# showlab/VideoSwap

Hardware: NVIDIA H100
Metric: denoise-steps/sec, 16f 512^2 SD1.5 UNet3D (CFG UNet fwd + CFG combine + DDIM step) (higher is better)
Workload: dtype f16

## Files before the change

### videoswap_b200/csrc/common.cuh

```cuda
#pragma once
#include <cuda.h>
#include <cuda_fp16.h>
#include <cuda_runtime.h>
#include <stdint.h>
#include <stdio.h>

namespace vs {

void set_error(const char* fmt, ...);
const char* last_error();

#define VS_CHECK_CUDA(expr)                                                                         \
  do {                                                                                              \
    cudaError_t _e = (expr);                                                                        \
    if (_e != cudaSuccess) {                                                                        \
      vs::set_error("%s:%d CUDA error %s: %s", __FILE__, __LINE__, #expr, cudaGetErrorString(_e)); \
      return 1;                                                                                     \
    }                                                                                               \
  } while (0)

#define VS_REQUIRE(cond, ...)                \
  do {                                       \
    if (!(cond)) {                           \
      vs::set_error(__VA_ARGS__);            \
      return 2;                              \
    }                                        \
  } while (0)

int make_tmap_f16(CUtensorMap* out, const void* base, int rank, const uint64_t* dims, const uint64_t* strides_bytes,
                  const uint32_t* box, int swizzle );

int num_sms();
int get_option(const char* name);

#ifdef __CUDACC__
template <typename... KArgs, typename... Args>
int launch_pdl(void (*kernel)(KArgs...), dim3 grid, dim3 block, size_t smem, cudaStream_t st, int cluster_x, Args&&... args) {
  cudaLaunchConfig_t cfg = {};
  cfg.gridDim = grid;
  cfg.blockDim = block;
  cfg.dynamicSmemBytes = smem;
  cfg.stream = st;
  cudaLaunchAttribute attr[2];
  int n = 0;
  if (get_option("pdl") != 0) {
    attr[n].id = cudaLaunchAttributeProgrammaticStreamSerialization;
    attr[n].val.programmaticStreamSerializationAllowed = 1;
    ++n;
  }
  if (cluster_x > 1) {
    attr[n].id = cudaLaunchAttributeClusterDimension;
    attr[n].val.clusterDim.x = cluster_x;
    attr[n].val.clusterDim.y = 1;
    attr[n].val.clusterDim.z = 1;
    ++n;
  }
  cfg.attrs = attr;
  cfg.numAttrs = n;
  VS_CHECK_CUDA(cudaLaunchKernelEx(&cfg, kernel, static_cast<KArgs>(args)...));
  return 0;
}
#endif

enum ProfCat { PC_GEMM = 0, PC_CONV = 1, PC_ATTN = 2, PC_TATTN = 3, PC_GROUPNORM = 4, PC_LAYERNORM = 5, PC_OTHER = 6, PC_COUNT = 7 };
struct ProfScope {
  ProfScope(cudaStream_t st, int cat, double work, int nlaunch = 1, long long m = 0, int n = 0, int k = 0);
  ~ProfScope();
  cudaStream_t st_; int idx_;
};
void prof_enable(bool on);
void prof_reset();
int prof_collect(int cat, double* ms, double* work, long long* count);
int prof_dump(const char* path);
long long launch_count();
void count_launch(int n);

#ifdef __CUDACC__
__device__ __forceinline__ uint32_t smem_u32(const void* p) { return (uint32_t)__cvta_generic_to_shared(p); }

__device__ __forceinline__ void mbar_init(uint32_t bar, uint32_t count) {
  asm volatile("mbarrier.init.shared::cta.b64 [%0], %1;" ::"r"(bar), "r"(count) : "memory");
}
__device__ __forceinline__ void fence_barrier_init() {
  asm volatile("fence.mbarrier_init.release.cluster;" ::: "memory");
}
__device__ __forceinline__ void fence_proxy_async() { asm volatile("fence.proxy.async.shared::cta;" ::: "memory"); }
__device__ __forceinline__ void mbar_expect_tx(uint32_t bar, uint32_t bytes) {
  asm volatile("mbarrier.arrive.expect_tx.shared::cta.b64 _, [%0], %1;" ::"r"(bar), "r"(bytes) : "memory");
}
__device__ __forceinline__ void mbar_arrive(uint32_t bar) {
  asm volatile("mbarrier.arrive.shared::cta.b64 _, [%0];" ::"r"(bar) : "memory");
}
__device__ __forceinline__ bool mbar_try_wait(uint32_t bar, uint32_t parity) {
  uint32_t ok;
  asm volatile(
      "{\n\t.reg .pred p;\n\t"
      "mbarrier.try_wait.parity.shared::cta.b64 p, [%1], %2;\n\t"
      "selp.u32 %0, 1, 0, p;\n\t}"
      : "=r"(ok)
      : "r"(bar), "r"(parity)
      : "memory");
  return ok != 0;
}
__device__ __forceinline__ void mbar_wait(uint32_t bar, uint32_t parity) {
  if (mbar_try_wait(bar, parity)) return;
  uint32_t spins = 0;
  while (!mbar_try_wait(bar, parity)) {
    if (++spins > (1u << 25)) __trap();
  }
}

__device__ __forceinline__ void prefetch_tmap(const CUtensorMap* m) {
  asm volatile("prefetch.tensormap [%0];" ::"l"(reinterpret_cast<uint64_t>(m)) : "memory");
}
__device__ __forceinline__ void tma_load_2d(uint32_t dst, const CUtensorMap* m, uint32_t bar, int c0, int c1) {
  asm volatile(
      "cp.async.bulk.tensor.2d.shared::cluster.global.mbarrier::complete_tx::bytes [%0], [%1, {%3, %4}], [%2];"
      ::"r"(dst), "l"(reinterpret_cast<uint64_t>(m)), "r"(bar), "r"(c0), "r"(c1)
      : "memory");
}
__device__ __forceinline__ void tma_load_4d(uint32_t dst, const CUtensorMap* m, uint32_t bar, int c0, int c1, int c2,
                                            int c3) {
  asm volatile(
      "cp.async.bulk.tensor.4d.shared::cluster.global.mbarrier::complete_tx::bytes [%0], [%1, {%3, %4, %5, %6}], [%2];"
      ::"r"(dst), "l"(reinterpret_cast<uint64_t>(m)), "r"(bar), "r"(c0), "r"(c1), "r"(c2), "r"(c3)
      : "memory");
}

__device__ __forceinline__ bool elect_one() {
  uint32_t pred;
  asm volatile(
      "{\n\t.reg .pred P;\n\t"
      "elect.sync _|P, 0xffffffff;\n\t"
      "selp.u32 %0, 1, 0, P;\n\t}"
      : "=r"(pred));
  return pred != 0;
}

__device__ __forceinline__ uint32_t cluster_ctarank() {
  uint32_t r;
  asm volatile("mov.u32 %0, %%cluster_ctarank;" : "=r"(r));
  return r;
}
__device__ __forceinline__ void cluster_sync_all() {
  asm volatile("barrier.cluster.arrive.release.aligned;" ::: "memory");
  asm volatile("barrier.cluster.wait.acquire.aligned;" ::: "memory");
}
__device__ __forceinline__ uint32_t mapa_shared(uint32_t addr, uint32_t rank) {
  uint32_t r;
  asm volatile("mapa.shared::cluster.u32 %0, %1, %2;" : "=r"(r) : "r"(addr), "r"(rank));
  return r;
}
__device__ __forceinline__ void named_bar_sync(int id, int nthreads) {
  asm volatile("bar.sync %0, %1;" ::"r"(id), "r"(nthreads) : "memory");
}
__device__ __forceinline__ void named_bar_arrive(int id, int nthreads) {
  asm volatile("bar.arrive %0, %1;" ::"r"(id), "r"(nthreads) : "memory");
}

__device__ __forceinline__ void pdl_trigger() { asm volatile("griddepcontrol.launch_dependents;" ::: "memory"); }
__device__ __forceinline__ void pdl_wait() { asm volatile("griddepcontrol.wait;" ::: "memory"); }

template <int N>
__device__ __forceinline__ void setmaxnreg_dec() { asm volatile("setmaxnreg.dec.sync.aligned.u32 %0;" ::"n"(N)); }
template <int N>
__device__ __forceinline__ void setmaxnreg_inc() { asm volatile("setmaxnreg.inc.sync.aligned.u32 %0;" ::"n"(N)); }

__device__ __forceinline__ void wgmma_fence() { asm volatile("wgmma.fence.sync.aligned;" ::: "memory"); }
__device__ __forceinline__ void wgmma_commit() { asm volatile("wgmma.commit_group.sync.aligned;" ::: "memory"); }
template <int N>
__device__ __forceinline__ void wgmma_wait() { asm volatile("wgmma.wait_group.sync.aligned %0;" ::"n"(N) : "memory"); }

__device__ __forceinline__ uint64_t gmma_desc_sw128(uint32_t smem_addr) {
  uint64_t d = 0;
  d |= (uint64_t)((smem_addr & 0x3FFFF) >> 4);
  d |= (uint64_t)1 << 16;
  d |= (uint64_t)(1024 >> 4) << 32;
  d |= (uint64_t)1 << 62;
  return d;
}
__device__ __forceinline__ uint64_t gmma_desc_sw128_mn(uint32_t smem_addr, uint32_t lbo_bytes) {
  uint64_t d = 0;
  d |= (uint64_t)((smem_addr & 0x3FFFF) >> 4);
  d |= (uint64_t)((lbo_bytes >> 4) & 0x3FFF) << 16;
  d |= (uint64_t)(1024 >> 4) << 32;
  d |= (uint64_t)1 << 62;
  return d;
}

#define VS_R8(i) "+f"(d[i]), "+f"(d[i + 1]), "+f"(d[i + 2]), "+f"(d[i + 3]), "+f"(d[i + 4]), "+f"(d[i + 5]), "+f"(d[i + 6]), "+f"(d[i + 7])
template <int N>
__device__ __forceinline__ void wgmma_ss(float* d, uint64_t da, uint64_t db, uint32_t scale_d);
#define VS_REGS_0_31 "%0,%1,%2,%3,%4,%5,%6,%7,%8,%9,%10,%11,%12,%13,%14,%15,%16,%17,%18,%19,%20,%21,%22,%23,%24,%25,%26,%27,%28,%29,%30,%31"
#define VS_REGS_32_63 "%32,%33,%34,%35,%36,%37,%38,%39,%40,%41,%42,%43,%44,%45,%46,%47,%48,%49,%50,%51,%52,%53,%54,%55,%56,%57,%58,%59,%60,%61,%62,%63"
#define VS_REGS_64_79 "%64,%65,%66,%67,%68,%69,%70,%71,%72,%73,%74,%75,%76,%77,%78,%79"
#define VS_REGS_80_127 "%80,%81,%82,%83,%84,%85,%86,%87,%88,%89,%90,%91,%92,%93,%94,%95,%96,%97,%98,%99,%100,%101,%102,%103,%104,%105,%106,%107,%108,%109,%110,%111,%112,%113,%114,%115,%116,%117,%118,%119,%120,%121,%122,%123,%124,%125,%126,%127"
#define VS_WGMMA_SS(N, REGS, IA, IB, IS, ...)                                                                     \
  template <>                                                                                                     \
  __device__ __forceinline__ void wgmma_ss<N>(float* d, uint64_t da, uint64_t db, uint32_t scale_d) {           \
    asm volatile("{\n\t.reg .pred p;\n\tsetp.ne.b32 p, %" #IS ", 0;\n\t"                                         \
                 "wgmma.mma_async.sync.aligned.m64n" #N "k16.f32.f16.f16 {" REGS "}, %" #IA ", %" #IB ", p, 1, 1, 0, 0;\n\t}" \
                 : __VA_ARGS__                                                                                    \
                 : "l"(da), "l"(db), "r"(scale_d));                                                               \
  }
VS_WGMMA_SS(64, VS_REGS_0_31, 32, 33, 34, VS_R8(0), VS_R8(8), VS_R8(16), VS_R8(24))
VS_WGMMA_SS(128, VS_REGS_0_31 "," VS_REGS_32_63, 64, 65, 66, VS_R8(0), VS_R8(8), VS_R8(16), VS_R8(24), VS_R8(32), VS_R8(40),
            VS_R8(48), VS_R8(56))
VS_WGMMA_SS(160, VS_REGS_0_31 "," VS_REGS_32_63 "," VS_REGS_64_79, 80, 81, 82, VS_R8(0), VS_R8(8), VS_R8(16), VS_R8(24),
            VS_R8(32), VS_R8(40), VS_R8(48), VS_R8(56), VS_R8(64), VS_R8(72))
VS_WGMMA_SS(256, VS_REGS_0_31 "," VS_REGS_32_63 "," VS_REGS_64_79 "," VS_REGS_80_127, 128, 129, 130, VS_R8(0), VS_R8(8),
            VS_R8(16), VS_R8(24), VS_R8(32), VS_R8(40), VS_R8(48), VS_R8(56), VS_R8(64), VS_R8(72), VS_R8(80), VS_R8(88),
            VS_R8(96), VS_R8(104), VS_R8(112), VS_R8(120))
#undef VS_WGMMA_SS
#undef VS_REGS_0_31
#undef VS_REGS_32_63
#undef VS_REGS_64_79
#undef VS_REGS_80_127
template <int TB = 0>
__device__ __forceinline__ void wgmma_m64n16(float* d, uint64_t da, uint64_t db, uint32_t scale_d) {
  asm volatile(
      "{\n\t.reg .pred p;\n\tsetp.ne.b32 p, %10, 0;\n\t"
      "wgmma.mma_async.sync.aligned.m64n16k16.f32.f16.f16 {%0,%1,%2,%3,%4,%5,%6,%7}, %8, %9, p, 1, 1, 0, %11;\n\t}"
      : VS_R8(0)
      : "l"(da), "l"(db), "r"(scale_d), "n"(TB));
}
template <int TB = 0>
__device__ __forceinline__ void wgmma_m64n64_rs(float* d, const uint32_t* a, uint64_t db, uint32_t scale_d) {
  asm volatile(
      "{\n\t.reg .pred p;\n\tsetp.ne.b32 p, %37, 0;\n\t"
      "wgmma.mma_async.sync.aligned.m64n64k16.f32.f16.f16 "
      "{%0,%1,%2,%3,%4,%5,%6,%7,%8,%9,%10,%11,%12,%13,%14,%15,%16,%17,%18,%19,%20,%21,%22,%23,%24,%25,%26,%27,%28,%29,%30,%31}, "
      "{%32,%33,%34,%35}, %36, p, 1, 1, %38;\n\t}"
      : VS_R8(0), VS_R8(8), VS_R8(16), VS_R8(24)
      : "r"(a[0]), "r"(a[1]), "r"(a[2]), "r"(a[3]), "l"(db), "r"(scale_d), "n"(TB));
}
template <int TB = 0>
__device__ __forceinline__ void wgmma_m64n16_rs(float* d, const uint32_t* a, uint64_t db, uint32_t scale_d) {
  asm volatile(
      "{\n\t.reg .pred p;\n\tsetp.ne.b32 p, %13, 0;\n\t"
      "wgmma.mma_async.sync.aligned.m64n16k16.f32.f16.f16 {%0,%1,%2,%3,%4,%5,%6,%7}, {%8,%9,%10,%11}, %12, p, 1, 1, %14;\n\t}"
      : VS_R8(0)
      : "r"(a[0]), "r"(a[1]), "r"(a[2]), "r"(a[3]), "l"(db), "r"(scale_d), "n"(TB));
}
#undef VS_R8

__device__ __forceinline__ float silu_f(float x) { return __fdividef(x, 1.f + __expf(-x)); }
__device__ __forceinline__ float gelu_erf_f(float x) { return 0.5f * x * (1.f + erff(x * 0.70710678118654752f)); }
__device__ __forceinline__ float gelu_erf_fast(float x) {
  const float z = fabsf(x) * 0.70710678118654752f;
  float t;
  asm("rcp.approx.ftz.f32 %0, %1;" : "=f"(t) : "f"(fmaf(0.3275911f, z, 1.f)));
  float poly = fmaf(1.061405429f, t, -1.453152027f);
  poly = fmaf(poly, t, 1.421413741f);
  poly = fmaf(poly, t, -0.284496736f);
  poly = fmaf(poly, t, 0.254829592f);
  poly *= t;
  float e;
  asm("ex2.approx.ftz.f32 %0, %1;" : "=f"(e) : "f"(-1.4426950408889634f * z * z));
  const float erf_abs = fmaf(-poly, e, 1.f);
  const float erf_s = copysignf(erf_abs, x);
  return 0.5f * x * (1.f + erf_s);
}
__device__ __forceinline__ float gelu_sig(float x) {
  const float xc = fminf(fmaxf(x, -5.f), 5.f);
  const float u = xc * xc;
  float q = fmaf(u, 2.47135360e-05f, 7.37690930e-04f);
  q = fmaf(q, u, -1.05988323e-01f);
  q = fmaf(q, u, -2.30164247e+00f);
  float e;
  asm("ex2.approx.ftz.f32 %0, %1;" : "=f"(e) : "f"(xc * q));
  return __fdividef(x, 1.f + e);
}
#endif

}
```

### videoswap_b200/csrc/gemm.cu

```cuda
#include "common.cuh"
#include "kernels.h"

namespace vs {

namespace {

constexpr int BM = 128;
constexpr int WG_M = 64;
constexpr int BK = 64;
constexpr int A_STAGE_BYTES = BM * BK * 2;
constexpr uint64_t A_HALF_DESC = (WG_M * BK * 2) >> 4;
constexpr int GEMM_THREADS = 384;
constexpr int SMEM_LIMIT = 227 * 1024;
constexpr int EPI_COLS = 32;
constexpr int EPI_WARP_BYTES = 16 * 64;
constexpr int EPI_BYTES = 8 * EPI_WARP_BYTES;
constexpr int PRODUCER_REGS = 40, CONSUMER_REGS = 232;
enum { EPI_F_GEGLU = 1, EPI_F_RES = 2, EPI_F_RV = 4, EPI_F_LN = 8, EPI_F_LNOUT = 16 };

struct GemmParams {
  CUtensorMap tmA, tmA2, tmB;
  int M, N;
  int num_kb;
  int kb_per_tap;
  int kb_src1;
  int taps;
  int a_rank;
  int nimg, H, W, TH, TW, TN, tiles_x, tiles_y;
  int tap_x0, tap_y0, tap_w;
  int osy, osx, ooy, oox, OH, OW;
  int tw_log, thw_log;
  int m_tiles, n_tiles;
  const float* bias;
  const float* rowvec;
  int ldrv;
  int pix_per_batch;
  int rv_mod;
  const float2* ln_stats;
  const float* ln_u;
  const float2* ln_parts;
  int ln_nparts;
  float ln_inv_c;
  float2* ln_sums_out;
  const __half* residual;
  int ldr;
  __half* out;
  int ldc;
  int staged;
  int stages;
};

template <int BN>
struct Cfg {
  static constexpr bool COOP = BN > 160;
  static constexpr int HALVES = COOP ? 1 : 2;
  static constexpr int B_STAGE_BYTES = BN * BK * 2;
  static constexpr int STAGE_BYTES = A_STAGE_BYTES + B_STAGE_BYTES;
  static constexpr int STAGES_RAW = (SMEM_LIMIT - 2048 - EPI_BYTES) / STAGE_BYTES;
  static constexpr int STAGES = STAGES_RAW > 12 ? 12 : STAGES_RAW;
  static constexpr int SMEM_BYTES = STAGES * STAGE_BYTES + EPI_BYTES + 1024  + 256 ;
  static_assert(B_STAGE_BYTES % 1024 == 0, "B stage must keep 1024-byte alignment for SWIZZLE_128B");
  static_assert(STAGES >= 3, "pipeline too shallow");
  static_assert(BN % 32 == 0 && BN <= 256, "wgmma N");
};

__device__ __forceinline__ uint32_t sw64_off(int row, int chunk) {
  return (uint32_t)(row * 64 + ((chunk ^ ((row >> 1) & 3)) << 4));
}

template <int BN, int EPI>
__global__ void __launch_bounds__(GEMM_THREADS, 1) gemm_tc_kernel(const __grid_constant__ GemmParams p) {
  using C = Cfg<BN>;
  constexpr bool GEGLU = (EPI & EPI_F_GEGLU) != 0, HAS_RES = (EPI & EPI_F_RES) != 0, HAS_RV = (EPI & EPI_F_RV) != 0;
  constexpr bool LN = (EPI & EPI_F_LN) != 0;
  constexpr bool LNOUT = (EPI & EPI_F_LNOUT) != 0;
  extern __shared__ uint8_t smem_raw[];
  const uint32_t smem_base = (smem_u32(smem_raw) + 1023u) & ~1023u;
  const uint32_t epi_base = smem_base + C::STAGES * C::STAGE_BYTES;
  const uint32_t bar_base = epi_base + EPI_BYTES;
  auto full_bar = [&](int s) { return bar_base + 8u * s; };
  auto empty_bar = [&](int s) { return bar_base + 8u * (C::STAGES + s); };

  const int warp = threadIdx.x >> 5;
  const int lane = threadIdx.x & 31;
  const int wg = threadIdx.x >> 7;
  const int nst = (p.stages > 0 && p.stages < C::STAGES) ? p.stages : C::STAGES;
  const int total_tiles = p.m_tiles * p.n_tiles;

  if (threadIdx.x == 0) {
    prefetch_tmap(&p.tmA);
    prefetch_tmap(&p.tmB);
    if (p.kb_src1 < p.kb_per_tap) prefetch_tmap(&p.tmA2);
    for (int s = 0; s < C::STAGES; ++s) {
      mbar_init(full_bar(s), 1);
      mbar_init(empty_bar(s), C::COOP ? 8 : 4);
    }
    fence_barrier_init();
  }
  __syncthreads();
  pdl_trigger();
  pdl_wait();

  if (wg == 0) {
    setmaxnreg_dec<PRODUCER_REGS>();
    if (warp != 0) return;
    const int num_kb = p.num_kb, kb_per_tap = p.kb_per_tap, kb_src1 = p.kb_src1;
    const bool conv = p.a_rank == 4;
    const int tap_x0 = p.tap_x0, tap_x1 = p.tap_x0 + p.tap_w;
    uint32_t pr_s = 0, pr_ph = 0;
    for (int t = blockIdx.x; t < total_tiles; t += gridDim.x) {
      const int m_tile = t / p.n_tiles, n_tile = t % p.n_tiles;
      int x0 = 0, y0 = 0, i0 = 0;
      if (conv) {
        x0 = (m_tile % p.tiles_x) * p.TW;
        y0 = ((m_tile / p.tiles_x) % p.tiles_y) * p.TH;
        i0 = (m_tile / (p.tiles_x * p.tiles_y)) * p.TN;
      }
      const int n0 = n_tile * BN;
      const int m0 = m_tile * BM;
      int kcoord = 0;
      int dy = p.tap_y0, dx = tap_x0;
      int r = 0;
      for (int kb = 0; kb < num_kb; ++kb) {
        mbar_wait(empty_bar(pr_s), pr_ph ^ 1);
        if (elect_one()) {
          const uint32_t fb = full_bar(pr_s);
          const uint32_t a_dst = smem_base + pr_s * C::STAGE_BYTES;
          const bool first = r < kb_src1;
          const CUtensorMap* tm = first ? &p.tmA : &p.tmA2;
          const int c = (first ? r : r - kb_src1) * BK;
          mbar_expect_tx(fb, C::STAGE_BYTES);
          if (conv) tma_load_4d(a_dst, tm, fb, c, x0 + dx, y0 + dy, i0);
          else tma_load_2d(a_dst, tm, fb, c, m0);
          tma_load_2d(a_dst + A_STAGE_BYTES, &p.tmB, fb, kcoord, n0);
        }
        __syncwarp();
        kcoord += BK;
        if (++r == kb_per_tap) {
          r = 0;
          if (++dx == tap_x1) { dx = tap_x0; ++dy; }
        }
        if (++pr_s == (uint32_t)nst) { pr_s = 0; pr_ph ^= 1; }
      }
    }
    return;
  }

  setmaxnreg_inc<CONSUMER_REGS>();
  const int g = wg - 1;
  const int wq = warp & 3;
  const int q = lane & 3;
  const int rbase = 16 * wq + (lane >> 2);
  const uint32_t stage_buf = epi_base + (uint32_t)(warp - 4) * EPI_WARP_BYTES;
  const bool has_bias = p.bias != nullptr;
  const bool staged = p.staged != 0;
  const int num_kb = p.num_kb;
  auto tile_pixel = [&](int m_tile, int row) -> int {
    if (p.a_rank == 4) {
      const int x0 = (m_tile % p.tiles_x) * p.TW;
      const int y0 = ((m_tile / p.tiles_x) % p.tiles_y) * p.TH;
      const int i0 = (m_tile / (p.tiles_x * p.tiles_y)) * p.TN;
      const int ti = row >> p.thw_log, rem = row & ((1 << p.thw_log) - 1);
      const int y = y0 + (rem >> p.tw_log), x = x0 + (rem & (p.TW - 1)), img = i0 + ti;
      return ((img < p.nimg) && (y < p.H) && (x < p.W)) ? (img * p.OH + y * p.osy + p.ooy) * p.OW + x * p.osx + p.oox : -1;
    }
    const int px = m_tile * BM + row;
    return px < p.M ? px : -1;
  };

  const int bar_mine = 1 + g, bar_other = 2 - g;
  float acc[C::HALVES][BN / 2];
  uint32_t s = 0, ph = 0;
  for (int t = blockIdx.x, j = 0; t < total_tiles; t += gridDim.x, ++j) {
    const int m_tile = t / p.n_tiles, n_tile = t % p.n_tiles;
    if (!C::COOP && (j & 1) != g) {
      const uint32_t sn = s + (uint32_t)num_kb;
      ph ^= (sn / (uint32_t)nst) & 1u;
      s = sn % (uint32_t)nst;
      continue;
    }
    if (!C::COOP && j > 0) named_bar_sync(bar_mine, 256);
    uint32_t prev = 0;
    for (int kb = 0; kb < num_kb; ++kb) {
      mbar_wait(full_bar(s), ph);
      wgmma_fence();
      const uint32_t a_addr = smem_base + s * C::STAGE_BYTES;
      const uint64_t da = gmma_desc_sw128(a_addr) + (C::COOP ? (uint64_t)g * A_HALF_DESC : 0);
      const uint64_t db = gmma_desc_sw128(a_addr + A_STAGE_BYTES);
#pragma unroll
      for (int k = 0; k < BK / 16; ++k) {
#pragma unroll
        for (int hh = 0; hh < C::HALVES; ++hh)
          wgmma_ss<BN>(acc[hh], da + hh * A_HALF_DESC + 2 * k, db + 2 * k, (kb | k) != 0 ? 1u : 0u);
      }
      wgmma_commit();
      if (kb > 0) {
        wgmma_wait<1>();
        if (lane == 0) mbar_arrive(empty_bar(prev));
      }
      prev = s;
      if (++s == (uint32_t)nst) { s = 0; ph ^= 1; }
    }
    if (!C::COOP && t + (int)gridDim.x < total_tiles) named_bar_arrive(bar_other, 256);
    wgmma_wait<0>();
    if (lane == 0) mbar_arrive(empty_bar(prev));

    const int n0 = n_tile * BN;
#pragma unroll
    for (int hh = 0; hh < C::HALVES; ++hh) {
      const int r0 = WG_M * (C::COOP ? g : hh) + rbase;
      int pix[2];
      pix[0] = tile_pixel(m_tile, r0);
      pix[1] = tile_pixel(m_tile, r0 + 8);
      const float* rv[2] = {nullptr, nullptr};
      if (HAS_RV || !staged) {
#pragma unroll
        for (int h = 0; h < 2; ++h) {
          if (p.rowvec != nullptr && pix[h] >= 0) {
            int ri = pix[h] / p.pix_per_batch;
            if (p.rv_mod > 0) ri %= p.rv_mod;
            rv[h] = p.rowvec + (long long)ri * p.ldrv + n0;
          }
        }
      }
      if (staged) {
        constexpr int OC = GEGLU ? BN / 2 : BN;
        const int oc0 = n_tile * OC;
        const int nsub = (p.N - n0 < BN ? (GEGLU ? (p.N - n0) / 2 : p.N - n0) : OC) / EPI_COLS;
        float la[2] = {1.f, 1.f}, lb[2] = {0.f, 0.f};
        if (LN) {
#pragma unroll
          for (int h = 0; h < 2; ++h) {
            if (pix[h] < 0) continue;
            if (p.ln_nparts > 0) {
              float S = 0.f, Q = 0.f;
              for (int k = 0; k < p.ln_nparts; ++k) {
                const float2 v = __ldg(p.ln_parts + (long long)k * p.M + pix[h]);
                S += v.x; Q += v.y;
              }
              const float mean = S * p.ln_inv_c;
              la[h] = rsqrtf(fmaxf(fmaf(-mean, mean, Q * p.ln_inv_c), 0.f) + 1e-5f);
              lb[h] = -mean * la[h];
            } else {
              const float2 st2 = __ldg(p.ln_stats + pix[h]);
              la[h] = st2.x; lb[h] = st2.y;
            }
          }
        }
        float rs[2] = {0.f, 0.f}, rq[2] = {0.f, 0.f};
        __half* orow[2];
        const __half* rrow[2];
#pragma unroll
        for (int h = 0; h < 2; ++h) {
          const long long px = pix[h] >= 0 ? pix[h] : 0;
          orow[h] = p.out + px * p.ldc + oc0 + q * 8;
          rrow[h] = HAS_RES ? p.residual + px * p.ldr + oc0 + q * 8 : nullptr;
        }
#pragma unroll
        for (int sb = 0; sb < OC / EPI_COLS; ++sb) {
          if (sb >= nsub) break;
          uint4 rr[2];
          if (HAS_RES) {
#pragma unroll
            for (int h = 0; h < 2; ++h) rr[h] = __ldg(reinterpret_cast<const uint4*>(rrow[h] + sb * EPI_COLS));
          }
#pragma unroll
          for (int jj = 0; jj < 4; ++jj) {
            const int j = 4 * sb + jj;
            const int c = 8 * j + 2 * q;
            float2 b = has_bias ? __ldg(reinterpret_cast<const float2*>(p.bias + n0 + c)) : make_float2(0.f, 0.f);
            float2 u = LN ? __ldg(reinterpret_cast<const float2*>(p.ln_u + n0 + c)) : make_float2(0.f, 0.f);
            float2 bg = make_float2(0.f, 0.f), ug = make_float2(0.f, 0.f);
            if (GEGLU) {
              bg = __ldg(reinterpret_cast<const float2*>(p.bias + n0 + BN / 2 + c));
              if (LN) ug = __ldg(reinterpret_cast<const float2*>(p.ln_u + n0 + BN / 2 + c));
            }
#pragma unroll
            for (int h = 0; h < 2; ++h) {
              float f0 = acc[hh][4 * j + 2 * h], f1 = acc[hh][4 * j + 2 * h + 1];
              if (GEGLU) {
                float g0 = acc[hh][4 * (j + BN / 16) + 2 * h], g1 = acc[hh][4 * (j + BN / 16) + 2 * h + 1];
                float bv0 = b.x, bv1 = b.y, bg0 = bg.x, bg1 = bg.y;
                if (LN) {
                  bv0 = fmaf(lb[h], u.x, bv0); bv1 = fmaf(lb[h], u.y, bv1);
                  bg0 = fmaf(lb[h], ug.x, bg0); bg1 = fmaf(lb[h], ug.y, bg1);
                  f0 *= la[h]; f1 *= la[h]; g0 *= la[h]; g1 *= la[h];
                }
                f0 = (f0 + bv0) * gelu_sig(g0 + bg0);
                f1 = (f1 + bv1) * gelu_sig(g1 + bg1);
              } else {
                if (LN) {
                  f0 = fmaf(la[h], f0, fmaf(lb[h], u.x, b.x));
                  f1 = fmaf(la[h], f1, fmaf(lb[h], u.y, b.y));
                } else if (has_bias) {
                  f0 += b.x; f1 += b.y;
                }
                if (HAS_RV && rv[h] != nullptr) {
                  const float2 r2 = __ldg(reinterpret_cast<const float2*>(rv[h] + c));
                  f0 += r2.x; f1 += r2.y;
                }
              }
              const __half2 hv = __floats2half2_rn(f0, f1);
              asm volatile("st.shared.b32 [%0], %1;" ::"r"(stage_buf + sw64_off((lane >> 2) + 8 * h, jj) + 4 * q),
                           "r"(*reinterpret_cast<const uint32_t*>(&hv)) : "memory");
            }
          }
          __syncwarp();
#pragma unroll
          for (int h = 0; h < 2; ++h) {
            uint4 o;
            asm volatile("ld.shared.v4.b32 {%0,%1,%2,%3}, [%4];" : "=r"(o.x), "=r"(o.y), "=r"(o.z), "=r"(o.w)
                         : "r"(stage_buf + sw64_off((lane >> 2) + 8 * h, q)));
            if (HAS_RES) {
              __half2* oh = reinterpret_cast<__half2*>(&o);
              const __half2* rh = reinterpret_cast<const __half2*>(&rr[h]);
#pragma unroll
              for (int t = 0; t < 4; ++t) oh[t] = __hadd2(oh[t], rh[t]);
            }
            if (pix[h] >= 0) *reinterpret_cast<uint4*>(orow[h] + sb * EPI_COLS) = o;
            if (LNOUT) {
              const __half2* oh = reinterpret_cast<const __half2*>(&o);
              const float2 a = __half22float2(oh[0]), b2 = __half22float2(oh[1]), c2 = __half22float2(oh[2]), d2 = __half22float2(oh[3]);
              rs[h] += ((a.x + a.y) + (b2.x + b2.y)) + ((c2.x + c2.y) + (d2.x + d2.y));
              float q0 = fmaf(a.x, a.x, a.y * a.y), q1 = fmaf(b2.x, b2.x, b2.y * b2.y);
              float q2 = fmaf(c2.x, c2.x, c2.y * c2.y), q3 = fmaf(d2.x, d2.x, d2.y * d2.y);
              rq[h] += (q0 + q1) + (q2 + q3);
            }
          }
          __syncwarp();
        }
        if (LNOUT) {
#pragma unroll
          for (int h = 0; h < 2; ++h) {
            rs[h] += __shfl_xor_sync(0xffffffffu, rs[h], 1); rq[h] += __shfl_xor_sync(0xffffffffu, rq[h], 1);
            rs[h] += __shfl_xor_sync(0xffffffffu, rs[h], 2); rq[h] += __shfl_xor_sync(0xffffffffu, rq[h], 2);
            if (q == 0 && pix[h] >= 0) p.ln_sums_out[(long long)n_tile * p.M + pix[h]] = make_float2(rs[h], rq[h]);
          }
        }
      } else {
#pragma unroll
        for (int j = 0; j < BN / 8; ++j) {
#pragma unroll
          for (int e = 0; e < 4; ++e) {
            const int h = e >> 1, c = 8 * j + 2 * q + (e & 1), n = n0 + c;
            if (n < p.N && pix[h] >= 0) {
              float f = acc[hh][4 * j + e];
              if (has_bias) f += p.bias[n];
              if (rv[h]) f += rv[h][c];
              if (p.residual) f += __half2float(p.residual[(long long)pix[h] * p.ldr + n]);
              p.out[(long long)pix[h] * p.ldc + n] = __float2half_rn(f);
            }
          }
        }
      }
    }
  }
}

struct ConvTile { int tw, th, tn; };

ConvTile pick_conv_tile(int nimg, int H, int W) {
  ConvTile best{1, 1, BM};
  long long best_cost = -1;
  for (int tw = 1; tw <= BM; tw *= 2) {
    for (int th = 1; tw * th <= BM; th *= 2) {
      const int tn = BM / (tw * th);
      if (tw > 256 || th > 256 || tn > 256) continue;
      const long long cost = (long long)((W + tw - 1) / tw) * tw * ((H + th - 1) / th) * th * ((nimg + tn - 1) / tn) * tn;
      if (best_cost < 0 || cost < best_cost || (cost == best_cost && tw > best.tw)) {
        best_cost = cost;
        best = ConvTile{tw, th, tn};
      }
    }
  }
  return best;
}

template <int BN, int EPI>
int launch(cudaStream_t st, const GemmParams& p) {
  using C = Cfg<BN>;
  static bool configured = false;
  if (!configured) {
    VS_CHECK_CUDA(cudaFuncSetAttribute(gemm_tc_kernel<BN, EPI>, cudaFuncAttributeMaxDynamicSharedMemorySize, C::SMEM_BYTES));
    configured = true;
  }
  const int total = p.m_tiles * p.n_tiles;
  int ctas = num_sms();
  const int cap = get_option("gemm_ctas");
  if (cap > 0 && cap < ctas) ctas = cap;
  return launch_pdl(gemm_tc_kernel<BN, EPI>, dim3(total < ctas ? total : ctas), dim3(GEMM_THREADS), C::SMEM_BYTES, st, 1, p);
}

template <int BN>
int launch_linear(cudaStream_t st, const GemmParams& p) {
  const int epi = (p.residual ? EPI_F_RES : 0) | (p.rowvec ? EPI_F_RV : 0) | ((p.ln_stats || p.ln_parts) ? EPI_F_LN : 0) |
                  (p.ln_sums_out ? EPI_F_LNOUT : 0);
  switch (epi) {
    case EPI_F_LNOUT: return launch<BN, EPI_F_LNOUT>(st, p);
    case EPI_F_LNOUT | EPI_F_RES: return launch<BN, EPI_F_LNOUT | EPI_F_RES>(st, p);
    case EPI_F_LN: return launch<BN, EPI_F_LN>(st, p);
    case EPI_F_LN | EPI_F_RV: return launch<BN, EPI_F_LN | EPI_F_RV>(st, p);
    case 0: return launch<BN, 0>(st, p);
    case EPI_F_RES: return launch<BN, EPI_F_RES>(st, p);
    case EPI_F_RV: return launch<BN, EPI_F_RV>(st, p);
    case EPI_F_RES | EPI_F_RV: return launch<BN, EPI_F_RES | EPI_F_RV>(st, p);
    default: set_error("gemm_tc: unsupported epilogue combination 0x%x", epi); return 2;
  }
}

int pick_bn(int m_tiles, int N, int num_kb) {
  if (N <= 64) return 64;
  int best = 128;
  long long best_cost = -1;
  const int cand[3] = {128, 160, 256};
  for (int i = 0; i < 3; ++i) {
    const int bn = cand[i];
    if (bn != 128 && N % bn != 0) continue;
    const long long tiles = (long long)m_tiles * ((N + bn - 1) / bn);
    const long long waves = (tiles + num_sms() - 1) / num_sms();
    const long long cost = waves * (16 + bn / 8);
    if (best_cost < 0 || cost < best_cost || (cost == best_cost && num_kb >= 40)) {
      best_cost = cost;
      best = bn;
    }
  }
  return best;
}

int ilog2(int v) { int l = 0; while ((1 << l) < v) ++l; return l; }

}

int gemm_n_tiles(const GemmArgs& a) {
  if (a.taps != 1) return 0;
  int bn = a.force_bn;
  if (a.mode == EPI_GEGLU) bn = 2 * kGegluGranule;
  else if (bn == 0) bn = pick_bn((a.M + BM - 1) / BM, a.N, (a.K1 + BK - 1) / BK + a.K2 / BK);
  return (a.N + bn - 1) / bn;
}

int gemm_tc(cudaStream_t st, const GemmArgs& a) {
  VS_REQUIRE(a.A && a.Bw && a.out, "gemm_tc: null pointer");
  VS_REQUIRE(a.taps == 1 || a.taps == 9 || a.taps == 4, "gemm_tc: taps must be 1, 9 (3x3) or 4 (2x2 sub-pixel)");
  VS_REQUIRE(a.K1 % 8 == 0 && a.K2 % 8 == 0, "gemm_tc: K must be a multiple of 8 (TMA 16-byte strides)");
  VS_REQUIRE((long long)a.M * (a.ldc > a.ldr ? a.ldc : a.ldr) < (1LL << 40) && a.M < (1 << 30), "gemm_tc: M too large");
  const bool two = a.A2 != nullptr && a.K2 > 0;
  if (two || a.taps != 1) VS_REQUIRE(a.K1 % BK == 0 && a.K2 % BK == 0, "gemm_tc: concat/conv sources need C %% 64 == 0 (got %d,%d)", a.K1, a.K2);
  GemmParams p;
  memset(&p, 0, sizeof(p));
  const int Ktap = a.K1 + (two ? a.K2 : 0);
  const int Ktot = Ktap * a.taps;
  p.taps = a.taps;
  p.kb_src1 = (a.K1 + BK - 1) / BK;
  p.kb_per_tap = p.kb_src1 + (two ? a.K2 / BK : 0);
  p.num_kb = p.kb_per_tap * a.taps;
  p.M = a.M;
  p.N = a.N;
  p.bias = a.bias;
  p.rowvec = a.rowvec;
  p.ldrv = a.ldrv > 0 ? a.ldrv : a.N;
  p.pix_per_batch = a.pix_per_batch > 0 ? a.pix_per_batch : 1;
  p.rv_mod = a.rv_mod;
  p.ln_stats = reinterpret_cast<const float2*>(a.ln_stats);
  p.ln_u = a.ln_u;
  p.ln_parts = reinterpret_cast<const float2*>(a.ln_parts);
  p.ln_nparts = a.ln_parts ? a.ln_nparts : 0;
  p.ln_inv_c = 1.f / (float)(a.K1 + a.K2);
  p.ln_sums_out = reinterpret_cast<float2*>(a.ln_sums_out);
  if (a.ln_parts) VS_REQUIRE(a.ln_stats == nullptr && a.ln_nparts >= 1 && a.ln_nparts <= 16 && a.taps == 1, "gemm_tc: bad LayerNorm partial-sum input");
  if (a.ln_stats || a.ln_parts) VS_REQUIRE(a.ln_u != nullptr && a.bias != nullptr && a.residual == nullptr, "gemm_tc: folded LayerNorm needs u and c vectors and no residual");
  if (a.ln_sums_out) VS_REQUIRE(a.taps == 1 && a.mode == EPI_LINEAR && a.rowvec == nullptr && !a.ln_stats && !a.ln_parts,
                                "gemm_tc: row statistics output is implemented for plain linear layers (+ bias / residual)");
  p.residual = a.residual;
  p.ldr = a.ldr;
  p.out = a.out;
  p.ldc = a.ldc;
  p.stages = get_option("gemm_stages");

  if (a.taps != 1) {
    VS_REQUIRE(a.nimg > 0 && a.H > 0 && a.W > 0 && a.M == a.nimg * a.H * a.W, "gemm_tc: bad conv geometry");
    p.a_rank = 4;
    if (a.taps == 9) { p.tap_x0 = p.tap_y0 = -1; p.tap_w = 3; p.osy = p.osx = 1; p.ooy = p.oox = 0; p.OH = a.H; p.OW = a.W; }
    else {
      VS_REQUIRE((a.sub_py | 1) == 1 && (a.sub_px | 1) == 1, "gemm_tc: sub-pixel parity must be 0 or 1");
      p.tap_y0 = a.sub_py - 1; p.tap_x0 = a.sub_px - 1; p.tap_w = 2;
      p.osy = p.osx = 2; p.ooy = a.sub_py; p.oox = a.sub_px; p.OH = 2 * a.H; p.OW = 2 * a.W;
    }
    const ConvTile t = pick_conv_tile(a.nimg, a.H, a.W);
    p.nimg = a.nimg; p.H = a.H; p.W = a.W; p.TW = t.tw; p.TH = t.th; p.TN = t.tn;
    p.tw_log = ilog2(t.tw);
    p.thw_log = ilog2(t.tw * t.th);
    p.tiles_x = (a.W + t.tw - 1) / t.tw;
    p.tiles_y = (a.H + t.th - 1) / t.th;
    p.m_tiles = p.tiles_x * p.tiles_y * ((a.nimg + t.tn - 1) / t.tn);
    const uint32_t box[4] = {BK, (uint32_t)t.tw, (uint32_t)t.th, (uint32_t)t.tn};
    {
      const uint64_t dims[4] = {(uint64_t)a.K1, (uint64_t)a.W, (uint64_t)a.H, (uint64_t)a.nimg};
      const uint64_t str[3] = {(uint64_t)a.lda1 * 2, (uint64_t)a.lda1 * 2 * a.W, (uint64_t)a.lda1 * 2 * a.W * a.H};
      if (make_tmap_f16(&p.tmA, a.A, 4, dims, str, box, 1)) return 3;
    }
    if (two) {
      const uint64_t dims[4] = {(uint64_t)a.K2, (uint64_t)a.W, (uint64_t)a.H, (uint64_t)a.nimg};
      const uint64_t str[3] = {(uint64_t)a.lda2 * 2, (uint64_t)a.lda2 * 2 * a.W, (uint64_t)a.lda2 * 2 * a.W * a.H};
      if (make_tmap_f16(&p.tmA2, a.A2, 4, dims, str, box, 1)) return 3;
    }
  } else {
    p.a_rank = 2;
    p.m_tiles = (a.M + BM - 1) / BM;
    const uint32_t box[2] = {BK, BM};
    {
      const uint64_t dims[2] = {(uint64_t)a.K1, (uint64_t)a.M};
      const uint64_t str[1] = {(uint64_t)a.lda1 * 2};
      if (make_tmap_f16(&p.tmA, a.A, 2, dims, str, box, 1)) return 3;
    }
    if (two) {
      const uint64_t dims[2] = {(uint64_t)a.K2, (uint64_t)a.M};
      const uint64_t str[1] = {(uint64_t)a.lda2 * 2};
      if (make_tmap_f16(&p.tmA2, a.A2, 2, dims, str, box, 1)) return 3;
    }
  }

  int bn = a.force_bn;
  if (a.mode == EPI_GEGLU) {
    bn = 2 * kGegluGranule;
    VS_REQUIRE(a.N % bn == 0, "gemm_tc: GEGLU needs N %% %d == 0 (N=%d)", bn, a.N);
    VS_REQUIRE(a.bias != nullptr && a.residual == nullptr && a.rowvec == nullptr, "gemm_tc: GEGLU takes a bias only");
  } else if (bn == 0) {
    bn = pick_bn(p.m_tiles, a.N, p.num_kb);
  }
  VS_REQUIRE(bn == 64 || bn == 128 || bn == 160 || bn == 256, "gemm_tc: unsupported BLOCK_N %d", bn);
  p.n_tiles = (a.N + bn - 1) / bn;
  {
    const uint64_t dims[2] = {(uint64_t)Ktot, (uint64_t)a.N};
    const uint64_t str[1] = {(uint64_t)Ktot * 2};
    const uint32_t box[2] = {BK, (uint32_t)bn};
    if (make_tmap_f16(&p.tmB, a.Bw, 2, dims, str, box, 1)) return 3;
  }
  const int out_cols = (a.mode == EPI_GEGLU) ? a.N / 2 : a.N;
  p.staged = (out_cols % EPI_COLS == 0) && (a.ldc % 8 == 0) && ((reinterpret_cast<uintptr_t>(a.out) & 15) == 0) &&
             (!a.residual || ((a.ldr % 8 == 0) && ((reinterpret_cast<uintptr_t>(a.residual) & 15) == 0))) &&
             (!a.bias || (reinterpret_cast<uintptr_t>(a.bias) & 15) == 0) &&
             (!a.rowvec || ((reinterpret_cast<uintptr_t>(a.rowvec) & 15) == 0 && p.ldrv % 4 == 0));
  if (!p.staged) VS_REQUIRE(a.mode == EPI_LINEAR, "gemm_tc: GEGLU output needs 32-column aligned, 16-byte strided rows");
  if (a.ln_stats || a.ln_parts) VS_REQUIRE(p.staged && (reinterpret_cast<uintptr_t>(a.ln_u) & 15) == 0, "gemm_tc: folded LayerNorm needs the staged epilogue");
  if (a.ln_sums_out) VS_REQUIRE(p.staged, "gemm_tc: row statistics output needs the staged epilogue (N %% 32 == 0, aligned rows)");
  ProfScope prof(st, a.taps != 1 ? PC_CONV : PC_GEMM, 2.0 * a.M * (double)a.N * Ktot, 1, a.M, a.N, Ktot);
  if (a.mode == EPI_GEGLU) {
    if (p.ln_stats || p.ln_parts) return launch<256, EPI_F_GEGLU | EPI_F_LN>(st, p);
    return launch<256, EPI_F_GEGLU>(st, p);
  }
  switch (bn) {
    case 64: return launch_linear<64>(st, p);
    case 128: return launch_linear<128>(st, p);
    case 256: return launch_linear<256>(st, p);
    default: return launch_linear<160>(st, p);
  }
}

}
```

Measured before the change: 8.513.

## Use TMA stores and TMA residual loads in GEMM epilogue with smem vector staging

Reworks the staged GEMM epilogue so each warpgroup writes its output tile into a swizzled shared-memory buffer and stores it with bulk TMA tensor stores. Residuals are prefetched by TMA into the same buffer before the mainloop finishes, and bias and LayerNorm vectors are staged in shared memory via cp.async. The aim is to replace scattered per-thread global stores and loads and overlap epilogue traffic with compute. In exchange, the larger epilogue buffers reduce pipeline stages, BN=256 is dropped from linear tile selection, and the async-proxy synchronisation becomes more complex.

```diff
diff --git a/videoswap_b200/csrc/common.cuh b/videoswap_b200/csrc/common.cuh
--- a/videoswap_b200/csrc/common.cuh
+++ b/videoswap_b200/csrc/common.cuh
@@ -126,6 +126,23 @@
       ::"r"(dst), "l"(reinterpret_cast<uint64_t>(m)), "r"(bar), "r"(c0), "r"(c1), "r"(c2), "r"(c3)
       : "memory");
 }
+__device__ __forceinline__ void tma_store_2d(const CUtensorMap* m, uint32_t src, int c0, int c1) {
+  asm volatile("cp.async.bulk.tensor.2d.global.shared::cta.bulk_group [%0, {%2, %3}], [%1];"
+               ::"l"(reinterpret_cast<uint64_t>(m)), "r"(src), "r"(c0), "r"(c1) : "memory");
+}
+__device__ __forceinline__ void tma_store_4d(const CUtensorMap* m, uint32_t src, int c0, int c1, int c2, int c3) {
+  asm volatile("cp.async.bulk.tensor.4d.global.shared::cta.bulk_group [%0, {%2, %3, %4, %5}], [%1];"
+               ::"l"(reinterpret_cast<uint64_t>(m)), "r"(src), "r"(c0), "r"(c1), "r"(c2), "r"(c3) : "memory");
+}
+__device__ __forceinline__ void bulk_commit() { asm volatile("cp.async.bulk.commit_group;" ::: "memory"); }
+template <int N>
+__device__ __forceinline__ void bulk_wait_read() { asm volatile("cp.async.bulk.wait_group.read %0;" ::"n"(N) : "memory"); }
+template <int N>
+__device__ __forceinline__ void bulk_wait() { asm volatile("cp.async.bulk.wait_group %0;" ::"n"(N) : "memory"); }
+__device__ __forceinline__ void cp_async16(uint32_t dst, const void* src) {
+  asm volatile("cp.async.cg.shared.global [%0], [%1], 16;" ::"r"(dst), "l"(src) : "memory");
+}
+__device__ __forceinline__ void cp_async_wait_all() { asm volatile("cp.async.wait_all;" ::: "memory"); }
 
 __device__ __forceinline__ bool elect_one() {
   uint32_t pred;
diff --git a/videoswap_b200/csrc/gemm.cu b/videoswap_b200/csrc/gemm.cu
--- a/videoswap_b200/csrc/gemm.cu
+++ b/videoswap_b200/csrc/gemm.cu
@@ -13,13 +13,14 @@
 constexpr int GEMM_THREADS = 384;
 constexpr int SMEM_LIMIT = 227 * 1024;
 constexpr int EPI_COLS = 32;
-constexpr int EPI_WARP_BYTES = 16 * 64;
-constexpr int EPI_BYTES = 8 * EPI_WARP_BYTES;
+constexpr int EPI_SUB_BYTES = WG_M * EPI_COLS * 2;
+constexpr int EPI_SLAB_BYTES = 16 * EPI_COLS * 2;
 constexpr int PRODUCER_REGS = 40, CONSUMER_REGS = 232;
 enum { EPI_F_GEGLU = 1, EPI_F_RES = 2, EPI_F_RV = 4, EPI_F_LN = 8, EPI_F_LNOUT = 16 };
 
 struct GemmParams {
   CUtensorMap tmA, tmA2, tmB;
+  CUtensorMap tmOut, tmRes;
   int M, N;
   int num_kb;
   int kb_per_tap;
@@ -50,15 +51,20 @@
   int stages;
 };
 
-template <int BN>
+template <int BN, int EPI>
 struct Cfg {
   static constexpr bool COOP = BN > 160;
   static constexpr int HALVES = COOP ? 1 : 2;
   static constexpr int B_STAGE_BYTES = BN * BK * 2;
   static constexpr int STAGE_BYTES = A_STAGE_BYTES + B_STAGE_BYTES;
-  static constexpr int STAGES_RAW = (SMEM_LIMIT - 2048 - EPI_BYTES) / STAGE_BYTES;
+  static constexpr int OC = (EPI & EPI_F_GEGLU) ? BN / 2 : BN;
+  static constexpr int OUT_BYTES = WG_M * OC * 2;
+  static constexpr int VEC_BYTES = COOP ? 0 : ((EPI & EPI_F_LN) ? 2 : 1) * BN * 4;
+  static constexpr int EPI_BYTES = 2 * (OUT_BYTES + VEC_BYTES);
+  static constexpr int STAGES_RAW = (SMEM_LIMIT - 1024 - 256 - EPI_BYTES) / STAGE_BYTES;
   static constexpr int STAGES = STAGES_RAW > 12 ? 12 : STAGES_RAW;
   static constexpr int SMEM_BYTES = STAGES * STAGE_BYTES + EPI_BYTES + 1024  + 256 ;
+  static_assert(SMEM_BYTES <= SMEM_LIMIT, "shared memory");
   static_assert(B_STAGE_BYTES % 1024 == 0, "B stage must keep 1024-byte alignment for SWIZZLE_128B");
   static_assert(STAGES >= 3, "pipeline too shallow");
   static_assert(BN % 32 == 0 && BN <= 256, "wgmma N");
@@ -70,14 +76,14 @@
 
 template <int BN, int EPI>
 __global__ void __launch_bounds__(GEMM_THREADS, 1) gemm_tc_kernel(const __grid_constant__ GemmParams p) {
-  using C = Cfg<BN>;
+  using C = Cfg<BN, EPI>;
   constexpr bool GEGLU = (EPI & EPI_F_GEGLU) != 0, HAS_RES = (EPI & EPI_F_RES) != 0, HAS_RV = (EPI & EPI_F_RV) != 0;
   constexpr bool LN = (EPI & EPI_F_LN) != 0;
   constexpr bool LNOUT = (EPI & EPI_F_LNOUT) != 0;
   extern __shared__ uint8_t smem_raw[];
   const uint32_t smem_base = (smem_u32(smem_raw) + 1023u) & ~1023u;
   const uint32_t epi_base = smem_base + C::STAGES * C::STAGE_BYTES;
-  const uint32_t bar_base = epi_base + EPI_BYTES;
+  const uint32_t bar_base = epi_base + C::EPI_BYTES;
   auto full_bar = [&](int s) { return bar_base + 8u * s; };
   auto empty_bar = [&](int s) { return bar_base + 8u * (C::STAGES + s); };
 
@@ -95,6 +101,7 @@
       mbar_init(full_bar(s), 1);
       mbar_init(empty_bar(s), C::COOP ? 8 : 4);
     }
+    for (int w = 0; w < 8; ++w) mbar_init(bar_base + 8u * (2 * C::STAGES + w), 1);
     fence_barrier_init();
   }
   __syncthreads();
@@ -148,15 +155,28 @@
 
   setmaxnreg_inc<CONSUMER_REGS>();
   const int g = wg - 1;
-  const int wq = warp & 3;
-  const int q = lane & 3;
-  const int rbase = 16 * wq + (lane >> 2);
-  const uint32_t stage_buf = epi_base + (uint32_t)(warp - 4) * EPI_WARP_BYTES;
+  struct Epi {
+    int q, rbase;
+    int row0;
+    bool leader;
+    uint32_t out_buf, slab, vec_buf, res_bar;
+    int bar;
+  };
+  auto epi_ctx = [&]() -> Epi {
+    uint32_t tx;
+    asm volatile("mov.u32 %0, %%tid.x;" : "=r"(tx));
+    const uint32_t cg = (tx >> 7) - 1u, wq4 = (tx >> 5) & 3;
+    const uint32_t ob = epi_base + cg * C::OUT_BYTES;
+    return Epi{(int)(tx & 3), (int)(16 * wq4 + ((tx & 31) >> 2)), (int)(16 * wq4), (tx & 31) == 0,
+               ob, ob + wq4 * EPI_SLAB_BYTES, epi_base + 2u * C::OUT_BYTES + cg * C::VEC_BYTES,
+               bar_base + 8u * (2 * C::STAGES + (tx >> 5) - 4), 3 + (int)cg};
+  };
   const bool has_bias = p.bias != nullptr;
   const bool staged = p.staged != 0;
+  const bool conv = p.a_rank == 4;
   const int num_kb = p.num_kb;
   auto tile_pixel = [&](int m_tile, int row) -> int {
-    if (p.a_rank == 4) {
+    if (conv) {
       const int x0 = (m_tile % p.tiles_x) * p.TW;
       const int y0 = ((m_tile / p.tiles_x) % p.tiles_y) * p.TH;
       const int i0 = (m_tile / (p.tiles_x * p.tiles_y)) * p.TN;
@@ -166,6 +186,37 @@
     }
     const int px = m_tile * BM + row;
     return px < p.M ? px : -1;
+  };
+  auto slab_tma = [&](bool store, const Epi& e, int m_tile, int oc0, int half, int nsub) {
+    const int r = WG_M * half + e.row0;
+    int c1 = m_tile * BM + r, c2 = 0, c3 = 0;
+    if (conv) {
+      c1 = (m_tile % p.tiles_x) * p.TW + (r & (p.TW - 1));
+      c2 = ((m_tile / p.tiles_x) % p.tiles_y) * p.TH + ((r >> p.tw_log) & (p.TH - 1));
+      c3 = (m_tile / (p.tiles_x * p.tiles_y)) * p.TN + (r >> p.thw_log);
+    }
+    if (!store) mbar_expect_tx(e.res_bar, (uint32_t)(nsub * EPI_SLAB_BYTES));
+    for (int sb = 0; sb < nsub; ++sb) {
+      const uint32_t sm = e.slab + sb * EPI_SUB_BYTES;
+      const int c0 = oc0 + sb * EPI_COLS;
+      if (store) {
+        if (conv) tma_store_4d(&p.tmOut, sm, c0, c1, c2, c3);
+        else tma_store_2d(&p.tmOut, sm, c0, c1);
+      } else {
+        if (conv) tma_load_4d(sm, &p.tmRes, e.res_bar, c0, c1, c2, c3);
+        else tma_load_2d(sm, &p.tmRes, e.res_bar, c0, c1);
+      }
+    }
+    if (store) bulk_commit();
+  };
+  auto vec2 = [&](const Epi& e, const float* gvec, int v, int c) -> float2 {
+    if constexpr (C::COOP) {
+      return __ldg(reinterpret_cast<const float2*>(gvec + c));
+    } else {
+      float2 r;
+      asm volatile("ld.shared.v2.f32 {%0,%1}, [%2];" : "=f"(r.x), "=f"(r.y) : "r"(e.vec_buf + 4u * (v * BN + c)));
+      return r;
+    }
   };
 
   const int bar_mine = 1 + g, bar_other = 2 - g;
@@ -179,7 +230,21 @@
       s = sn % (uint32_t)nst;
       continue;
     }
+    auto tile_cols = [&](int& n0, int& oc0, int& nsub) {
+      n0 = n_tile * BN;
+      oc0 = n_tile * C::OC;
+      nsub = (p.N - n0 < BN ? (GEGLU ? (p.N - n0) / 2 : p.N - n0) : C::OC) / EPI_COLS;
+    };
     if (!C::COOP && j > 0) named_bar_sync(bar_mine, 256);
+    if (staged) {
+      int n0, oc0, nsub;
+      tile_cols(n0, oc0, nsub);
+      const Epi e = epi_ctx();
+      if (HAS_RES && e.leader) {
+        bulk_wait_read<0>();
+        slab_tma(false, e, m_tile, oc0, C::COOP ? g : 0, nsub);
+      }
+    }
     uint32_t prev = 0;
     for (int kb = 0; kb < num_kb; ++kb) {
       mbar_wait(full_bar(s), ph);
@@ -202,16 +267,47 @@
       if (++s == (uint32_t)nst) { s = 0; ph ^= 1; }
     }
     if (!C::COOP && t + (int)gridDim.x < total_tiles) named_bar_arrive(bar_other, 256);
+    int n0, oc0, nsub;
+    tile_cols(n0, oc0, nsub);
+    const Epi e = epi_ctx();
+    const int q = e.q, rbase = e.rbase;
+    if (!C::COOP && staged) {
+      constexpr int CH = BN / 4;
+      const int i = threadIdx.x & 127;
+      if (i < (LN ? 2 : 1) * CH) {
+        const int v = i / CH, col = n0 + 4 * (i % CH);
+        const float* src = v ? p.ln_u : p.bias;
+        if (src != nullptr && col < p.N) cp_async16(e.vec_buf + 16u * i, src + col);
+      }
+    }
     wgmma_wait<0>();
     if (lane == 0) mbar_arrive(empty_bar(prev));
-
-    const int n0 = n_tile * BN;
+    if (!C::COOP && staged) cp_async_wait_all();
+
 #pragma unroll
     for (int hh = 0; hh < C::HALVES; ++hh) {
       const int r0 = WG_M * (C::COOP ? g : hh) + rbase;
       int pix[2];
-      pix[0] = tile_pixel(m_tile, r0);
-      pix[1] = tile_pixel(m_tile, r0 + 8);
+      float la[2] = {1.f, 1.f}, lb[2] = {0.f, 0.f};
+#pragma unroll
+      for (int h = 0; h < 2; ++h) {
+        pix[h] = tile_pixel(m_tile, r0 + 8 * h);
+        if (LN && pix[h] >= 0) {
+          if (p.ln_nparts > 0) {
+            float S = 0.f, Q = 0.f;
+            for (int k = 0; k < p.ln_nparts; ++k) {
+              const float2 v = __ldg(p.ln_parts + (long long)k * p.M + pix[h]);
+              S += v.x; Q += v.y;
+            }
+            const float mean = S * p.ln_inv_c;
+            la[h] = rsqrtf(fmaxf(fmaf(-mean, mean, Q * p.ln_inv_c), 0.f) + 1e-5f);
+            lb[h] = -mean * la[h];
+          } else {
+            const float2 st2 = __ldg(p.ln_stats + pix[h]);
+            la[h] = st2.x; lb[h] = st2.y;
+          }
+        }
+      }
       const float* rv[2] = {nullptr, nullptr};
       if (HAS_RV || !staged) {
 #pragma unroll
@@ -224,56 +320,28 @@
         }
       }
       if (staged) {
-        constexpr int OC = GEGLU ? BN / 2 : BN;
-        const int oc0 = n_tile * OC;
-        const int nsub = (p.N - n0 < BN ? (GEGLU ? (p.N - n0) / 2 : p.N - n0) : OC) / EPI_COLS;
-        float la[2] = {1.f, 1.f}, lb[2] = {0.f, 0.f};
-        if (LN) {
-#pragma unroll
-          for (int h = 0; h < 2; ++h) {
-            if (pix[h] < 0) continue;
-            if (p.ln_nparts > 0) {
-              float S = 0.f, Q = 0.f;
-              for (int k = 0; k < p.ln_nparts; ++k) {
-                const float2 v = __ldg(p.ln_parts + (long long)k * p.M + pix[h]);
-                S += v.x; Q += v.y;
-              }
-              const float mean = S * p.ln_inv_c;
-              la[h] = rsqrtf(fmaxf(fmaf(-mean, mean, Q * p.ln_inv_c), 0.f) + 1e-5f);
-              lb[h] = -mean * la[h];
-            } else {
-              const float2 st2 = __ldg(p.ln_stats + pix[h]);
-              la[h] = st2.x; lb[h] = st2.y;
-            }
-          }
-        }
-        float rs[2] = {0.f, 0.f}, rq[2] = {0.f, 0.f};
-        __half* orow[2];
-        const __half* rrow[2];
-#pragma unroll
-        for (int h = 0; h < 2; ++h) {
-          const long long px = pix[h] >= 0 ? pix[h] : 0;
-          orow[h] = p.out + px * p.ldc + oc0 + q * 8;
-          rrow[h] = HAS_RES ? p.residual + px * p.ldr + oc0 + q * 8 : nullptr;
-        }
-#pragma unroll
-        for (int sb = 0; sb < OC / EPI_COLS; ++sb) {
+        const int half = C::COOP ? g : hh;
+        if (e.leader) {
+          bulk_wait_read<0>();
+          if (HAS_RES && hh > 0) slab_tma(false, e, m_tile, oc0, half, nsub);
+        }
+        if (!C::COOP && hh == 0) named_bar_sync(e.bar, 128);
+        else __syncwarp();
+        if (HAS_RES) mbar_wait(e.res_bar, C::COOP ? (uint32_t)j & 1u : (uint32_t)hh);
+#pragma unroll
+        for (int sb = 0; sb < C::OC / EPI_COLS; ++sb) {
           if (sb >= nsub) break;
-          uint4 rr[2];
-          if (HAS_RES) {
-#pragma unroll
-            for (int h = 0; h < 2; ++h) rr[h] = __ldg(reinterpret_cast<const uint4*>(rrow[h] + sb * EPI_COLS));
-          }
+          const uint32_t sub = e.out_buf + sb * EPI_SUB_BYTES;
 #pragma unroll
           for (int jj = 0; jj < 4; ++jj) {
             const int j = 4 * sb + jj;
             const int c = 8 * j + 2 * q;
-            float2 b = has_bias ? __ldg(reinterpret_cast<const float2*>(p.bias + n0 + c)) : make_float2(0.f, 0.f);
-            float2 u = LN ? __ldg(reinterpret_cast<const float2*>(p.ln_u + n0 + c)) : make_float2(0.f, 0.f);
+            float2 b = has_bias ? vec2(e, p.bias + n0, 0, c) : make_float2(0.f, 0.f);
+            float2 u = LN ? vec2(e, p.ln_u + n0, 1, c) : make_float2(0.f, 0.f);
             float2 bg = make_float2(0.f, 0.f), ug = make_float2(0.f, 0.f);
             if (GEGLU) {
-              bg = __ldg(reinterpret_cast<const float2*>(p.bias + n0 + BN / 2 + c));
-              if (LN) ug = __ldg(reinterpret_cast<const float2*>(p.ln_u + n0 + BN / 2 + c));
+              bg = vec2(e, p.bias + n0, 0, BN / 2 + c);
+              if (LN) ug = vec2(e, p.ln_u + n0, 1, BN / 2 + c);
             }
 #pragma unroll
             for (int h = 0; h < 2; ++h) {
@@ -300,25 +368,28 @@
                   f0 += r2.x; f1 += r2.y;
                 }
               }
-              const __half2 hv = __floats2half2_rn(f0, f1);
-              asm volatile("st.shared.b32 [%0], %1;" ::"r"(stage_buf + sw64_off((lane >> 2) + 8 * h, jj) + 4 * q),
-                           "r"(*reinterpret_cast<const uint32_t*>(&hv)) : "memory");
+              __half2 hv = __floats2half2_rn(f0, f1);
+              const uint32_t addr = sub + sw64_off(rbase + 8 * h, jj) + 4 * q;
+              if (HAS_RES) {
+                uint32_t r;
+                asm volatile("ld.shared.b32 %0, [%1];" : "=r"(r) : "r"(addr));
+                hv = __hadd2(hv, *reinterpret_cast<const __half2*>(&r));
+              }
+              asm volatile("st.shared.b32 [%0], %1;" ::"r"(addr), "r"(*reinterpret_cast<const uint32_t*>(&hv)));
             }
           }
+        }
+        if (LNOUT) {
           __syncwarp();
-#pragma unroll
-          for (int h = 0; h < 2; ++h) {
-            uint4 o;
-            asm volatile("ld.shared.v4.b32 {%0,%1,%2,%3}, [%4];" : "=r"(o.x), "=r"(o.y), "=r"(o.z), "=r"(o.w)
-                         : "r"(stage_buf + sw64_off((lane >> 2) + 8 * h, q)));
-            if (HAS_RES) {
-              __half2* oh = reinterpret_cast<__half2*>(&o);
-              const __half2* rh = reinterpret_cast<const __half2*>(&rr[h]);
-#pragma unroll
-              for (int t = 0; t < 4; ++t) oh[t] = __hadd2(oh[t], rh[t]);
-            }
-            if (pix[h] >= 0) *reinterpret_cast<uint4*>(orow[h] + sb * EPI_COLS) = o;
-            if (LNOUT) {
+          float rs[2] = {0.f, 0.f}, rq[2] = {0.f, 0.f};
+#pragma unroll
+          for (int sb = 0; sb < C::OC / EPI_COLS; ++sb) {
+            if (sb >= nsub) break;
+#pragma unroll
+            for (int h = 0; h < 2; ++h) {
+              uint4 o;
+              asm volatile("ld.shared.v4.b32 {%0,%1,%2,%3}, [%4];" : "=r"(o.x), "=r"(o.y), "=r"(o.z), "=r"(o.w)
+                           : "r"(e.out_buf + sb * EPI_SUB_BYTES + sw64_off(rbase + 8 * h, q)));
               const __half2* oh = reinterpret_cast<const __half2*>(&o);
               const float2 a = __half22float2(oh[0]), b2 = __half22float2(oh[1]), c2 = __half22float2(oh[2]), d2 = __half22float2(oh[3]);
               rs[h] += ((a.x + a.y) + (b2.x + b2.y)) + ((c2.x + c2.y) + (d2.x + d2.y));
@@ -327,15 +398,18 @@
               rq[h] += (q0 + q1) + (q2 + q3);
             }
           }
-          __syncwarp();
-        }
-        if (LNOUT) {
 #pragma unroll
           for (int h = 0; h < 2; ++h) {
             rs[h] += __shfl_xor_sync(0xffffffffu, rs[h], 1); rq[h] += __shfl_xor_sync(0xffffffffu, rq[h], 1);
             rs[h] += __shfl_xor_sync(0xffffffffu, rs[h], 2); rq[h] += __shfl_xor_sync(0xffffffffu, rq[h], 2);
             if (q == 0 && pix[h] >= 0) p.ln_sums_out[(long long)n_tile * p.M + pix[h]] = make_float2(rs[h], rq[h]);
           }
+        }
+        fence_proxy_async();
+        __syncwarp();
+        if (e.leader) {
+          slab_tma(true, e, m_tile, oc0, half, nsub);
+          if (hh == C::HALVES - 1 && t + (C::COOP ? 1 : 2) * (int)gridDim.x >= total_tiles) bulk_wait<0>();
         }
       } else {
 #pragma unroll
@@ -378,7 +452,7 @@
 
 template <int BN, int EPI>
 int launch(cudaStream_t st, const GemmParams& p) {
-  using C = Cfg<BN>;
+  using C = Cfg<BN, EPI>;
   static bool configured = false;
   if (!configured) {
     VS_CHECK_CUDA(cudaFuncSetAttribute(gemm_tc_kernel<BN, EPI>, cudaFuncAttributeMaxDynamicSharedMemorySize, C::SMEM_BYTES));
@@ -412,8 +486,8 @@
   if (N <= 64) return 64;
   int best = 128;
   long long best_cost = -1;
-  const int cand[3] = {128, 160, 256};
-  for (int i = 0; i < 3; ++i) {
+  const int cand[2] = {128, 160};
+  for (int i = 0; i < 2; ++i) {
     const int bn = cand[i];
     if (bn != 128 && N % bn != 0) continue;
     const long long tiles = (long long)m_tiles * ((N + bn - 1) / bn);
@@ -544,6 +618,28 @@
   if (!p.staged) VS_REQUIRE(a.mode == EPI_LINEAR, "gemm_tc: GEGLU output needs 32-column aligned, 16-byte strided rows");
   if (a.ln_stats || a.ln_parts) VS_REQUIRE(p.staged && (reinterpret_cast<uintptr_t>(a.ln_u) & 15) == 0, "gemm_tc: folded LayerNorm needs the staged epilogue");
   if (a.ln_sums_out) VS_REQUIRE(p.staged, "gemm_tc: row statistics output needs the staged epilogue (N %% 32 == 0, aligned rows)");
+  if (p.staged) {
+    if (a.taps != 1) {
+      uint32_t hb[3];
+      hb[0] = p.TW < 16 ? p.TW : 16;
+      hb[1] = (uint32_t)p.TH < 16 / hb[0] ? p.TH : 16 / hb[0];
+      hb[2] = 16 / (hb[0] * hb[1]);
+      const uint32_t box[4] = {EPI_COLS, hb[0], hb[1], hb[2]};
+      const uint64_t dims[4] = {(uint64_t)out_cols, (uint64_t)a.W, (uint64_t)a.H, (uint64_t)a.nimg};
+      auto map = [&](CUtensorMap* m, const __half* base, int ld) {
+        const uint64_t str[3] = {(uint64_t)ld * 2 * p.osx, (uint64_t)ld * 2 * p.osy * p.OW, (uint64_t)ld * 2 * p.OW * p.OH};
+        return make_tmap_f16(m, base + (long long)(p.ooy * p.OW + p.oox) * ld, 4, dims, str, box, 2);
+      };
+      if (map(&p.tmOut, a.out, a.ldc)) return 3;
+      if (a.residual && map(&p.tmRes, a.residual, a.ldr)) return 3;
+    } else {
+      const uint32_t box[2] = {EPI_COLS, 16};
+      const uint64_t dims[2] = {(uint64_t)out_cols, (uint64_t)a.M};
+      const uint64_t str_o[1] = {(uint64_t)a.ldc * 2}, str_r[1] = {(uint64_t)a.ldr * 2};
+      if (make_tmap_f16(&p.tmOut, a.out, 2, dims, str_o, box, 2)) return 3;
+      if (a.residual && make_tmap_f16(&p.tmRes, a.residual, 2, dims, str_r, box, 2)) return 3;
+    }
+  }
   ProfScope prof(st, a.taps != 1 ? PC_CONV : PC_GEMM, 2.0 * a.M * (double)a.N * Ktot, 1, a.M, a.N, Ktot);
   if (a.mode == EPI_GEGLU) {
     if (p.ln_stats || p.ln_parts) return launch<256, EPI_F_GEGLU | EPI_F_LN>(st, p);
```

Measured after the change: 8.597, median of 6. No clear change (+1.0%).
